# openvinotoolkit/openvino_tokenizers

Hardware: AMD Instinct MI355X
Metric: input MB/s encoded (GPT-2 BPE, 512-byte strings) (higher is better)
Workload: dtype u8/int32

## Files before the change

openvino_tokenizers_amd/csrc/api_common.hpp:

```cpp
#pragma once

#include <atomic>
#include <cstdio>
#include <cstdlib>
#include <functional>

#include <hip/hip_runtime.h>

#include <algorithm>
#include <string>

#include "encode_kernels.hpp"
#include "regex_device.hpp"
#include "runtime.hpp"
#include "tables.hpp"

struct ovtk_regex_split {
    int device = 0;
    ovtk::SplitDev dev{};
    int mode = 1;
    bool invert = false;
    int max_splits = -1;
    ovtk::RegexDev regex{};
    ovtk::DevBuf r_trans, r_ascii, r_index, r_blocks, r_ctx;
// ... 479 lines not shown
                                                                : op_ + ": output ids buffer too small (" + std::to_string(st.n_out) +
                                                                      " ids, capacity " + std::to_string(out_.data_capacity) + ")");
                if (wire_.hdr || dense_on_) return OVTK_OK;
                if (direct_out_) return OVTK_OK;
                if (int rc = copy_back(out_.begins, d_begins_, size_t(n_rows_) * 4, mem_, s_)) return rc;
                if (int rc = copy_back(out_.ends, d_ends_, size_t(n_rows_) * 4, mem_, s_)) return rc;
                if (int rc = copy_back(out_.data, d_ids_, size_t(st.n_out) * 4, mem_, s_)) return rc;
                if (mem_ == OVTK_MEM_HOST) OVTK_HIP(hipStreamSynchronize(s_));
                return OVTK_OK;
            }
            small_ = false;
            if (int rc = launch()) return rc;
        }
        return set_error(OVTK_E_HIP, "workspace sizing did not converge");
    }

private:
    int launch() {
        OVTK_HIP(hipSetDevice(device_));
        Workspace& ws = *ws_.ws;
        int e = 0;
        e = e ? e : ws.row_stage.ensure(size_t(n_rows_) * 4);
        e = e ? e : ws.row_cnt.ensure(size_t(n_rows_) * 4);
        e = e ? e : ws.row_used.ensure(size_t(n_rows_) * 4);
        e = e ? e : ws.stage.ensure(size_t(stage_cap_) * 4 + 64);
        e = e ? e : ws.deferred.ensure(size_t(shard_cap_) * kShards * sizeof(DeferredPiece));
        e = e ? e : ws.exact.ensure(size_t(exact_cap_) * sizeof(ExactPiece));
        e = e ? e : ws.scratch.ensure(size_t(scratch_cap_));
        e = e ? e : ws.wave_off.ensure(size_t(grid_ * kWavesPerBlock + 1) * sizeof(long long));
        e = e ? e : ws.tiles.ensure(size_t(n_tiles_ + 1) * sizeof(long long));
        const bool fold = fold_tail_ && n_rows_ <= kFoldTailRows;
        size_t status_bytes = sizeof(RunStatus) + (fold ? size_t(n_tiles_) * 4 + 16 : 0);
        const int sp_mode = plan_.short_path_mode;
        small_ = small_ && !(plan_.short_ok && sp_mode == 2);
        const bool span_sums = plan_.short_ok && !small_ && fold && !force_long_;
        const size_t status_stride = (status_bytes + 255) & ~size_t(255);
        e = e ? e : ws.status.ensure(2 * status_stride);
        if (fold) e = e ? e : ws.gen[4].ensure(size_t(n_rows_) * 4);
        if (self_alloc_) e = e ? e : ws.gen[5].ensure(size_t(n_rows_) * 4);
        if (e) return e;
        EncodeWork w{};
        w.n_waves = grid_ * kWavesPerBlock;
        w.fold_tail = fold;
        uint8_t* const status_base = ws.status.as<uint8_t>();
        w.tile_cnt = fold ? reinterpret_cast<int32_t*>(status_base + sizeof(RunStatus)) : nullptr;
        w.row_emit = fold ? ws.gen[4].as<int32_t>() : nullptr;
        w.pending_rows = self_alloc_ ? ws.gen[5].as<int32_t>() : nullptr;
        w.out_cap = out_.data_capacity;
        w.rows_per_ticket = plan_.rows_per_ticket;
        w.wave_off = self_alloc_ ? nullptr : ws.wave_off.as<long long>();
        w.stage_region = int32_t(stage_cap_ / kShards);
        w.row_stage = ws.row_stage.as<int32_t>();
        w.row_cnt = ws.row_cnt.as<int32_t>();
        w.row_used = ws.row_used.as<int32_t>();
        w.tile_off = ws.tiles.as<long long>();
        w.stage = ws.stage.as<int32_t>();
        w.stage_cap = int32_t(stage_cap_);
        w.stage16 = plan_.stage16 ? 1 : 0;
        w.deferred = ws.deferred.as<DeferredPiece>();
        w.shard_cap = int32_t(std::min<int64_t>(shard_cap_, INT32_MAX / kShards));
        w.exact = ws.exact.as<ExactPiece>();
        w.exact_cap = int32_t(exact_cap_);
        w.scratch = ws.scratch.as<uint8_t>();
        w.scratch_cap = uint32_t(std::min<int64_t>(scratch_cap_, 0xFFFFFFF0ll));
        w.status = ws.status.as<RunStatus>();
        phase_ = 0;

        if (small_ && fold) {
            w.small = 1;
            const int blocks = std::max(1, std::min((n_rows_ + kWavesPerBlock - 1) / kWavesPerBlock, kSmallRows / kWavesPerBlock));
            w.n_waves = blocks * kWavesPerBlock;
            w.out_ids = d_ids_;
            w.out_begins = d_begins_;
            w.out_ends = d_ends_;
            w.host_status = ws.host_status;
            w.status_words = int32_t(status_bytes / 4);
            if (ws.clean_status != w.status || ws.clean_bytes < status_bytes || ws.clean_after_lease + 1 != ws.lease_count)
                OVTK_HIP(hipMemsetAsync(w.status, 0, status_bytes, s_));
            ws.clean_status = nullptr;
            pending_clean_ = w.status;
            pending_clean_bytes_ = status_bytes;
            std::memset(ws.host_status, 0, sizeof(RunStatus));
            ws.host_status->flags = kFlagDidNotRun;
            middle_(ws, d_in_, w, blocks);
            OVTK_HIP(hipEventRecord(ws.done, s_));
            return OVTK_OK;
        }
        ws.clean_status = nullptr;
        ws.status_half ^= 1;
        uint8_t* mine = status_base + size_t(ws.status_half) * status_stride;
        uint8_t* other = status_base + size_t(ws.status_half ^ 1) * status_stride;
        w.status = reinterpret_cast<RunStatus*>(mine);
        w.tile_cnt = fold ? reinterpret_cast<int32_t*>(mine + sizeof(RunStatus)) : nullptr;
        w.next_status = reinterpret_cast<RunStatus*>(other);
        w.tile_sums = fold && (n_tiles_ <= kTileSumTiles || span_sums) ? 1 : 0;
        w.host_status = ws.host_status;
        w.status_words = int32_t(status_bytes / 4);
        if (ws.zeroed_status != mine || ws.zeroed_bytes < status_bytes || ws.zeroed_after_lease + 1 != ws.lease_count)
            OVTK_HIP(hipMemsetAsync(w.status, 0, status_bytes, s_));
        ws.zeroed_status = nullptr;
        std::memset(ws.host_status, 0, sizeof(RunStatus));
        ws.host_status->flags = kFlagDidNotRun;
        if (!self_alloc_)
            OVTK_LAUNCH(ws.marks, "prep_rows", prep_rows_kernel, std::min(grid_, kTicketBlocks), kBlockThreads, s_, d_in_, mul_, w);
        w.launch_mask = kLaunchAll;
        if (span_sums) {
            w.span_sums = 1;
            w.skip_mask = sp_mode == 2 ? (kSkipPending | kSkipMerge) : ((expect_pending_ ? 0 : kSkipPending) | (expect_merge_ ? 0 : kSkipMerge));
            w.launch_mask = kLaunchSpan | ((w.skip_mask & kSkipPending) ? 0 : kLaunchPending) | ((w.skip_mask & kSkipMerge) ? 0 : kLaunchMerge);
            w.merge_hint = int32_t(std::min<int64_t>(merge_hint_, INT32_MAX));
            w_ = w;
            phase_ = 1;
        }
        middle_(ws, d_in_, w, grid_);
        return launch_tail(ws, w, other, status_bytes);
    }

    int launch_phase2(const RunStatus& st) {
        OVTK_HIP(hipSetDevice(device_));
        Workspace& ws = *ws_.ws;
        const bool pending_now = (w_.skip_mask & kSkipPending) && st.n_pending > 0;
        if (pending_now && !(w_.skip_mask & kSkipMerge)) {
            force_long_ = true;
            return launch();
        }
        EncodeWork w = w_;
        w.merge_hint = st.n_unresolved;
        w.launch_mask = (pending_now ? kLaunchPending : 0) | ((w_.skip_mask & kSkipMerge) ? kLaunchMerge : 0);
        w.skip_mask = pending_now || !(w_.skip_mask & kSkipPending) ? 0 : kSkipPending;
        static_assert(offsetof(RunStatus, width_ticket) == offsetof(RunStatus, width) + 4, "width and width_ticket are cleared together");
        OVTK_HIP(hipMemsetAsync(&w.status->width, 0, 8, s_));
        OVTK_HIP(hipMemsetAsync(&w.status->flags, 0, 4, s_));
        OVTK_HIP(hipMemsetAsync(&w.status->n_out, 0, 4, s_));
        std::memset(ws.host_status, 0, sizeof(RunStatus));
        ws.host_status->flags = kFlagDidNotRun;
        middle_(ws, d_in_, w, grid_);
        phase_ = 2;
        return launch_tail(ws, w, zeroed_other_, zeroed_other_bytes_);
    }

    int launch_tail(Workspace& ws, EncodeWork& w, const void* other, size_t status_bytes) {
        if (!w.fold_tail)
            OVTK_LAUNCH(ws.marks, "count_scan", count_scan_kernel, std::min((n_tiles_ + 3) / 4, kTicketBlocks), kBlockThreads, s_,
                        n_rows_, w, (long long)out_.data_capacity);
        int split = 1;
        if (!dense_on_ && !wire_.hdr) {
            const long long ids_per_item = (long long)kCompactRows * (in_.strings.n_chars / std::max<long long>(1, n_rows_)) / 4;
            while (split < 16 && ids_per_item >= 2048ll * split && (long long)(n_rows_ / kCompactRows) * split * 2 <= std::max<long long>((long long)device_cu_count(device_) * 64, 1024)) split *= 2;
        }
        w.compact_split = split;
        const long long units = ((long long)n_rows_ + kCompactRows - 1) / kCompactRows * split;
        const int cgrid = int(std::max<long long>(1, std::min<long long>((units + kWavesPerBlock - 1) / kWavesPerBlock, (long long)device_cu_count(device_) * 16)));
        const RaggedSink rsink{d_ids_, d_begins_, d_ends_};
        with_bool(plan_.stage16, [&](auto s16) {
            constexpr bool S16 = decltype(s16)::value;
            if (pair_on_) {
                PairDenseSink pair = pair_;
                pair.row_cnt = w.row_cnt;
                pair.n = n_rows_ / 2;
                OVTK_LAUNCH(ws.marks, "pair_width", pair_width_kernel, std::min(64, (pair.n + kBlockThreads - 1) / kBlockThreads), kBlockThreads, s_, n_rows_, w, pair);
                OVTK_LAUNCH(ws.marks, "compact", (compact_kernel<PairDenseSink, S16>), cgrid, kBlockThreads, s_, n_rows_, w, pair);
            } else if (dense_on_) {
                OVTK_LAUNCH(ws.marks, "row_width", row_width_kernel, std::min(64, (n_rows_ + kBlockThreads - 1) / kBlockThreads), kBlockThreads, s_, n_rows_, w, dense_);
                OVTK_LAUNCH(ws.marks, "compact", (compact_kernel<DenseSink, S16>), cgrid, kBlockThreads, s_, n_rows_, w, dense_);
            } else if (wire_.hdr) OVTK_LAUNCH(ws.marks, "compact", (compact_kernel<WireSink, S16>), cgrid, kBlockThreads, s_, n_rows_, w, wire_);
            else OVTK_LAUNCH(ws.marks, "compact", (compact_kernel<RaggedSink, S16>), cgrid, kBlockThreads, s_, n_rows_, w, rsink);
        });
        pending_zeroed_ = other;
        pending_zeroed_bytes_ = status_bytes;
        zeroed_other_ = other;
        zeroed_other_bytes_ = status_bytes;
        OVTK_HIP(hipEventRecord(ws.done, s_));
        return OVTK_OK;
    }

    int device_;
    std::string op_;
    ovtk_ragged_strings in_;
    const uint8_t* skips_;
    int mul_;
    ovtk_ragged_i32_out out_;
    int mem_, in_mem_;
    bool direct_out_ = false;
    std::shared_ptr<void> keep_;
    std::vector<std::shared_ptr<WorkspaceLease>> others_;
    std::function<int()> front_check_;
    hipStream_t s_;
    Middle middle_;
    bool self_alloc_;
    EncodePlan plan_;
    WorkspaceLease ws_;
    bool fold_tail_;
    bool small_ok_ = false, small_ = false;
    bool expect_pending_ = false, expect_merge_ = true, force_long_ = false;
    int64_t merge_hint_ = -1;
    int phase_ = 0;
    EncodeWork w_{};
    const void* zeroed_other_ = nullptr;
    size_t zeroed_other_bytes_ = 0;
    const void* pending_zeroed_ = nullptr;
    size_t pending_zeroed_bytes_ = 0;
    const void* pending_clean_ = nullptr;
    size_t pending_clean_bytes_ = 0;
    WireSink wire_{};
    DenseSink dense_{};
    bool dense_on_ = false;
    PairDenseSink pair_{};
    bool pair_on_ = false;
    std::function<void(const RunStatus&)> on_status_;
    RowsIn d_in_{};
    int n_rows_ = 0, grid_ = 0, n_tiles_ = 0;
    int64_t stage_cap_ = 0, shard_cap_ = 0, exact_cap_ = 0, scratch_cap_ = 0;
    int32_t *d_begins_ = nullptr, *d_ends_ = nullptr, *d_ids_ = nullptr;
};

template <class Middle>
std::unique_ptr<RowsRun<std::decay_t<Middle>>> make_rows_run(int device, const char* op, const ovtk_ragged_strings* in,
                                                             const uint8_t* skips, int mul, const ovtk_ragged_i32_out* out, int mem,
                                                             hipStream_t s, Middle&& middle, const EncodePlan* plan = nullptr) {
    return std::make_unique<RowsRun<std::decay_t<Middle>>>(device, op, in, skips, mul, out, mem, s, std::forward<Middle>(middle), plan);
}

inline int pair_sink_from_params(const char* op, const ovtk_ragged_strings* in, int64_t n_first, const ovtk_pair_dense_params* p, int32_t* out_ids,
                                 uint8_t* out_mask, int32_t* out_type_ids, int64_t capacity, PairDenseSink& d) {
    const std::string name(op);
    if (!p || !out_ids || !in || capacity < 0) return set_error(OVTK_E_ARG, name + ": null argument");
    if (n_first < 0 || in->n_rows - n_first != n_first)
        return set_error(OVTK_E_ARG, name + ": the one call takes as many second rows as first ones (" + std::to_string(n_first) + " + " +
                                         std::to_string(in->n_rows - n_first) +
                                         "); 1 against n or an empty second input: the two-call form (the encode on all rows, then ovtk_encode_tail_run over the halves)");
    if (p->n_front < 0 || p->n_between < 0 || p->n_behind < 0 || (p->n_front && !p->front) || (p->n_between && !p->between) ||
        (p->n_behind && !p->behind) || p->max_length < 0)
        return set_error(OVTK_E_ARG, name + ": bad constant ids or max_length < 0");
    if (p->n_front > kDenseAffix || p->n_between > kDenseAffix || p->n_behind > kDenseAffix)
        return set_error(OVTK_E_UNSUPPORTED, name + ": at most 4 constant ids in front / between / behind");
    if (p->trunc_mode < 0 || p->trunc_mode > 2) return set_error(OVTK_E_ARG, name + ": Unknown truncation mode: " + std::to_string(p->trunc_mode));
    d = PairDenseSink{};
    d.ids = out_ids;
    d.mask = out_mask;
    d.types = out_type_ids;
    d.capacity = capacity;
    d.n = int32_t(n_first);
    d.max_length = p->max_length;
    d.trunc_left = p->trunc_left ? 1 : 0;
    d.mode = p->trunc_mode;
    d.pad_right = p->pad_right ? 1 : 0;
    d.pad_value = p->pad_value;
    d.type_pad = p->type_pad_value;
    d.target_dim = p->target_dim;
    d.n_front = p->n_front;
    d.n_between = p->n_between;
    d.n_behind = p->n_behind;
    for (int i = 0; i < d.n_front; ++i) d.front[i] = p->front[i];
    for (int i = 0; i < d.n_between; ++i) d.between[i] = p->between[i];
    for (int i = 0; i < d.n_behind; ++i) d.behind[i] = p->behind[i];
    for (int i = 0; i < 5; ++i) d.type_ids[i] = p->type_ids[i];
    return OVTK_OK;
}
inline int pair_rows_without_text(const PairDenseSink& d, int device, hipStream_t s, ovtk_pending& p) {
    const int32_t len = d.n_front + d.n_between + d.n_behind, T = d.target_dim >= 0 ? d.target_dim : (d.n > 0 ? len : 0);
    *p.dense_width = T;
    if (int64_t(d.n) * T > d.capacity) {
        p.late_rc = OVTK_E_CAPACITY;
        p.late_msg = "encode_pair_dense: dense outputs too small (row width " + std::to_string(T) + ")";
        return OVTK_OK;
    }
    if (T <= 0 || d.n <= 0) return OVTK_OK;
    const size_t cells = size_t(d.n) * size_t(T);
    std::vector<int32_t> ids(cells, d.pad_value), types(d.types ? cells : 0, d.type_pad);
    std::vector<uint8_t> mask(d.mask ? cells : 0, 0);
    const int col0 = d.pad_right ? 0 : std::max(0, T - len);
    for (int64_t r = 0; r < d.n; ++r)
        for (int k = 0; k < len && col0 + k < T; ++k) {
            const bool f = k < d.n_front, b = !f && k < d.n_front + d.n_between;
            const size_t at = size_t(r) * size_t(T) + size_t(col0 + k);
            ids[at] = f ? d.front[k] : (b ? d.between[k - d.n_front] : d.behind[k - d.n_front - d.n_between]);
            if (d.types) types[at] = f ? d.type_ids[0] : (b ? d.type_ids[2] : d.type_ids[4]);
            if (d.mask) mask[at] = 1;
        }
    OVTK_HIP(hipSetDevice(device));
    OVTK_HIP(hipMemcpyAsync(d.ids, ids.data(), cells * 4, hipMemcpyHostToDevice, s));
    if (d.mask) OVTK_HIP(hipMemcpyAsync(d.mask, mask.data(), cells, hipMemcpyHostToDevice, s));
    if (d.types) OVTK_HIP(hipMemcpyAsync(d.types, types.data(), cells * 4, hipMemcpyHostToDevice, s));
    OVTK_HIP(hipStreamSynchronize(s));
    return OVTK_OK;
}

template <class Middle>
int run_rows_to_ids(int device, const char* op, const ovtk_ragged_strings* in, const uint8_t* skips, int mul,
                    ovtk_ragged_i32_out* out, int mem, hipStream_t s, Middle&& middle) {
    auto run = make_rows_run(device, op, in, skips, mul, out, mem, s, std::forward<Middle>(middle));
    if (int rc = run->start()) return rc;
    return run->finish(out);
}

}
```

openvino_tokenizers_amd/csrc/encode_kernels.hpp:

```cpp
#pragma once

#include <cstddef>
#include <type_traits>

#include "bpe_device.hpp"
#include "device_common.hpp"
#include "scan_kernels.hpp"
#include "split_device.hpp"
#include "split_seq_device.hpp"

namespace ovtk {

struct RowsIn {
    const int32_t* ragged_begins;
    const int32_t* ragged_ends;
    int32_t n_rows;
    const int32_t* begins;
    const int32_t* ends;
    int32_t n_strings;
    const uint8_t* chars;
    int64_t n_chars;
    const uint8_t* skips;
};

// ... 1211 lines not shown
        }
    }
    __device__ __forceinline__ void finish(int, const RunStatus*) const {}
};
static __global__ __launch_bounds__(kBlockThreads) void row_width_kernel(int n_rows, EncodeWork w, DenseSink d) {
    int m = 0;
    if (d.target_dim < 0) {
        for (int r = int(blockIdx.x) * kBlockThreads + int(threadIdx.x); r < n_rows; r += int(gridDim.x) * kBlockThreads) {
            const int c = w.row_cnt[r];
            const int len = (c < d.max_length ? c : d.max_length) + d.n_pre + d.n_suf;
            m = len > m ? len : m;
        }
        m = wave_max(m);
        if (lane_id() == 0 && m > 0) atomicMax(&w.status->width, m);
    } else if (blockIdx.x == 0 && threadIdx.x == 0) {
        w.status->width = d.target_dim;
    }
    if (!last_block_done(&w.status->width_ticket, gridDim.x, false)) return;
    if (threadIdx.x == 0) {
        const int T = __hip_atomic_load(&w.status->width, __ATOMIC_RELAXED, __HIP_MEMORY_SCOPE_AGENT);
        if ((long long)T * n_rows > d.capacity) atomicOr(&w.status->flags, kFlagOutCapacity);
    }
}
struct PairDenseSink {
    int32_t* ids;
    uint8_t* mask;
    int32_t* types;
    int64_t capacity;
    const int32_t* row_cnt;
    int32_t n;
    int32_t max_length;
    int32_t trunc_left;
    int32_t mode;
    int32_t pad_right, pad_value, type_pad;
    int32_t target_dim;
    int32_t n_front, n_between, n_behind;
    int32_t front[kDenseAffix], between[kDenseAffix], behind[kDenseAffix];
    int32_t type_ids[5];
    int32_t T;
    __device__ __forceinline__ void start(const RunStatus* st) { T = st->width; }
    __device__ __forceinline__ int32_t front_at(int k) const { return k == 0 ? front[0] : (k == 1 ? front[1] : (k == 2 ? front[2] : front[3])); }
    __device__ __forceinline__ int32_t between_at(int k) const { return k == 0 ? between[0] : (k == 1 ? between[1] : (k == 2 ? between[2] : between[3])); }
    __device__ __forceinline__ int32_t behind_at(int k) const { return k == 0 ? behind[0] : (k == 1 ? behind[1] : (k == 2 ? behind[2] : behind[3])); }
    __device__ __forceinline__ void kept(int32_t fl, int32_t sl, int32_t& keep_f, int32_t& keep_s) const {
        const int32_t m = max_length;
        keep_f = fl;
        keep_s = sl;
        if (fl + sl > m) {
            const int32_t half = m / 2, half_up = m / 2 + m % 2;
            if (mode == 0) keep_f = fl > m ? m : fl;
            else if (mode == 1) keep_s = sl > m ? m : sl;
            else if (fl >= half_up && sl <= half) keep_f = m - sl;
            else if (fl < half_up && sl > half) keep_s = m - fl;
            else {
                keep_f = half + (m % 2) * (fl >= sl);
                keep_s = half + (m % 2) * (fl < sl);
            }
        }
    }
    __device__ __forceinline__ int col0_of(int len) const { return pad_right ? 0 : (T > len ? T - len : 0); }
    __device__ __forceinline__ void row(int, int, int) const {}
    __device__ __forceinline__ void id(int r, int cnt, int j, int, int32_t v) const {
        const bool second = r >= n;
        const int i = second ? r - n : r;
        const int32_t other = row_cnt[second ? i : r + n];
        int32_t kf, ks;
        kept(second ? other : cnt, second ? cnt : other, kf, ks);
        const int keep = second ? ks : kf, first = trunc_left ? cnt - keep : 0;
        if (j < first || j >= first + keep) return;
        const int len = n_front + kf + n_between + ks + n_behind;
        const int col = col0_of(len) + n_front + (second ? kf + n_between : 0) + (j - first);
        if (col < T) ids[(long long)i * T + col] = v;
    }
    __device__ __forceinline__ void row_done(int r, int cnt) const {
        if (r >= n) return;
        int32_t kf, ks;
        kept(cnt, row_cnt[r + n], kf, ks);
        const int a1 = n_front, a2 = a1 + kf, a3 = a2 + n_between, a4 = a3 + ks, len = a4 + n_behind;
        const int col0 = col0_of(len);
        for (int c = lane_id(); c < T; c += kWave) {
            const int k = c - col0;
            const bool inside = k >= 0 && k < len;
            const long long at = (long long)r * T + c;
            if (mask) mask[at] = inside ? uint8_t(1) : uint8_t(0);
            if (types)
                types[at] = !inside ? type_pad
                                    : (k < a1 ? type_ids[0] : (k < a2 ? type_ids[1] : (k < a3 ? type_ids[2] : (k < a4 ? type_ids[3] : type_ids[4]))));
            if (!inside) ids[at] = pad_value;
            else if (k < a1) ids[at] = front_at(k);
            else if (k >= a2 && k < a3) ids[at] = between_at(k - a2);
            else if (k >= a4) ids[at] = behind_at(k - a4);
        }
    }
    __device__ __forceinline__ void finish(int, const RunStatus*) const {}
};
static __global__ __launch_bounds__(kBlockThreads) void pair_width_kernel(int n_rows, EncodeWork w, PairDenseSink d) {
    const int n = n_rows / 2;
    int m = 0;
    if (d.target_dim < 0) {
        for (int r = int(blockIdx.x) * kBlockThreads + int(threadIdx.x); r < n; r += int(gridDim.x) * kBlockThreads) {
            int32_t kf, ks;
            d.kept(w.row_cnt[r], w.row_cnt[r + n], kf, ks);
            const int len = d.n_front + kf + d.n_between + ks + d.n_behind;
            m = len > m ? len : m;
        }
        m = wave_max(m);
        if (lane_id() == 0 && m > 0) atomicMax(&w.status->width, m);
    } else if (blockIdx.x == 0 && threadIdx.x == 0) {
        w.status->width = d.target_dim;
    }
    if (!last_block_done(&w.status->width_ticket, gridDim.x, false)) return;
    if (threadIdx.x == 0) {
        const int T = __hip_atomic_load(&w.status->width, __ATOMIC_RELAXED, __HIP_MEMORY_SCOPE_AGENT);
        if ((long long)T * n > d.capacity) atomicOr(&w.status->flags, kFlagOutCapacity);
    }
}
template <class Sink>
struct is_dense_sink { static constexpr bool value = std::is_same<Sink, DenseSink>::value || std::is_same<Sink, PairDenseSink>::value; };
struct WireSink {
    int32_t* hdr;
    int32_t* ends;
    void* ids;
    int32_t pad_ids, max_rows, id_bytes;
    __device__ __forceinline__ void start(const RunStatus*) {}
    __device__ __forceinline__ void row(int r, int, int e) const { ends[r] = e; }
    __device__ __forceinline__ void row_done(int, int) const {}
    __device__ __forceinline__ void id(int, int, int, int pos, int32_t v) const {
        if (pos >= pad_ids) return;
        if (id_bytes == 2) static_cast<uint16_t*>(ids)[pos] = uint16_t(v);
        else static_cast<int32_t*>(ids)[pos] = v;
    }
    __device__ __forceinline__ void finish(int n_rows, const RunStatus* st) const {
        if (blockIdx.x != 0) return;
        if (threadIdx.x == 0) {
            hdr[0] = st->n_out;
            hdr[1] = n_rows;
            hdr[2] = hdr[3] = 0;
        }
        for (int r = n_rows + int(threadIdx.x); r < max_rows; r += kBlockThreads) ends[r] = 0;
    }
};

template <bool S16>
__device__ __forceinline__ int32_t stage_get_t(const EncodeWork& w, int pos) {
    if (S16) {
        const uint32_t x = reinterpret_cast<const uint16_t*>(w.stage)[pos];
        return x == 0xFFFFu ? kEmptyId : int32_t(x);
    }
    return w.stage[pos];
}
constexpr int kFlatIds = kWave * 8;
struct __attribute__((packed, aligned(1))) FlatBytes16 { uint32_t d[4]; };
struct __attribute__((packed, aligned(1))) FlatBytes8 { uint32_t d[2]; };
template <bool S16>
__device__ __forceinline__ void flat_copy(const uint8_t* stage_bytes, int total_used, bool plain, int32_t* out, int32_t* buf, int part, int split) {
    constexpr int E = S16 ? 8 : 4;
    const int l = lane_id();
    auto fetch = [&](int off) -> FlatBytes16 {
        const int idx = off + l * E;
        if (idx < total_used) return *reinterpret_cast<const FlatBytes16*>(stage_bytes + idx * (S16 ? 2 : 4));
        return FlatBytes16{{0u, 0u, 0u, 0u}};
    };
    if (plain) {
        constexpr int U = 2;
        for (int off0 = part * (U * kWave * 4); off0 < total_used; off0 += split * (U * kWave * 4)) {
            uint32_t x[U][4];
#pragma unroll
            for (int u = 0; u < U; ++u) {
                const int idx = off0 + (u * kWave + l) * 4;
                x[u][0] = x[u][1] = x[u][2] = x[u][3] = 0u;
                if (idx < total_used) {
                    if (S16) {
                        const FlatBytes8 r = *reinterpret_cast<const FlatBytes8*>(stage_bytes + idx * 2);
                        x[u][0] = r.d[0] & 0xFFFFu; x[u][1] = r.d[0] >> 16; x[u][2] = r.d[1] & 0xFFFFu; x[u][3] = r.d[1] >> 16;
                    } else {
                        const FlatBytes16 r = *reinterpret_cast<const FlatBytes16*>(stage_bytes + idx * 4);
                        x[u][0] = r.d[0]; x[u][1] = r.d[1]; x[u][2] = r.d[2]; x[u][3] = r.d[3];
                    }
                }
            }
#pragma unroll
            for (int u = 0; u < U; ++u) {
                const int idx = off0 + (u * kWave + l) * 4;
                const int n_here = total_used - idx;
                if (n_here >= 4) {
                    *reinterpret_cast<FlatBytes16*>(out + idx) = FlatBytes16{{x[u][0], x[u][1], x[u][2], x[u][3]}};
                } else {
                    if (n_here > 0) out[idx] = int32_t(x[u][0]);
                    if (n_here > 1) out[idx + 1] = int32_t(x[u][1]);
                    if (n_here > 2) out[idx + 2] = int32_t(x[u][2]);
                }
            }
        }
        return;
    }
    FlatBytes16 v = fetch(0);
    for (int off = 0; off < total_used; off += kWave * E) {
        const FlatBytes16 nxt = fetch(off + kWave * E);
        const int n_here = total_used - (off + l * E);
        int32_t e[E];
        uint32_t valid = 0;
#pragma unroll
        for (int i = 0; i < E; ++i) {
            if (S16) {
                const uint32_t x = (v.d[i >> 1] >> (16 * (i & 1))) & 0xFFFFu;
                e[i] = int32_t(x);
                if (i < n_here && x != 0xFFFFu) valid |= 1u << i;
            } else {
                e[i] = int32_t(v.d[i]);
                if (i < n_here && e[i] != kEmptyId) valid |= 1u << i;
            }
        }
        const int c = __popc(valid);
        const int incl = wave_incl_sum(c);
        int at = incl - c;
#pragma unroll
        for (int i = 0; i < E; ++i)
            if ((valid >> i) & 1u) buf[at++] = e[i];
        const int total = wave_readlane(incl, kWave - 1);
        wave_sync();
        for (int t = 4 * l; t < total; t += 4 * kWave) {
            if (t + 4 <= total) {
                *reinterpret_cast<FlatBytes16*>(out + t) = *reinterpret_cast<const FlatBytes16*>(buf + t);
            } else {
                for (int i = t; i < total; ++i) out[i] = buf[i];
            }
        }
        out += total;
        v = nxt;
        wave_sync();
    }
}
template <bool S16>
__device__ __forceinline__ bool compact_flat(const EncodeWork& w, const RaggedSink& sink, int32_t* buf, const int (&cnt)[4], const int (&o)[4],
                                             const int (&base)[4], const int (&used)[4], int row0, int part, int split) {
    const int l = lane_id();
    const int total_used = used[0] + used[1] + used[2] + used[3];
    if (used[0] < 0 || used[1] < 0 || used[2] < 0 || used[3] < 0 || base[1] != base[0] + used[0] || base[2] != base[1] + used[1] ||
        base[3] != base[2] + used[2])
        return false;
    const bool plain = total_used == cnt[0] + cnt[1] + cnt[2] + cnt[3];
    if (part != 0 && !plain) return true;
    if (l < 4 && part == 0) {
        const int oo = l == 0 ? o[0] : (l == 1 ? o[1] : (l == 2 ? o[2] : o[3])), cc = l == 0 ? cnt[0] : (l == 1 ? cnt[1] : (l == 2 ? cnt[2] : cnt[3]));
        sink.row(row0 + l, oo, oo + cc);
    }
    flat_copy<S16>(reinterpret_cast<const uint8_t*>(w.stage) + (long long)base[0] * (S16 ? 2 : 4), total_used, plain, sink.ids + o[0], buf, part, split);
    return true;
}

template <class Sink, bool S16 = false>
__device__ __forceinline__ void compact_body(int n_rows, const EncodeWork& w, Sink sink, bool solo = false, int32_t* flat_buf = nullptr,
                                             uint32_t more_flags = 0u) {
    if ((w.status->flags | more_flags) & (kFatalFlags | kFlagOutCapacity | kFlagDeferOverflow | kFlagExactOverflow | kFlagScratchOverflow |
                                         kFlagTailPending))
        return;
    if ((w.skip_mask & kSkipPending) && w.status->n_pending != 0) return;
    if (w.skip_mask & kSkipMerge) {
        const int mine = lane_id() < kShards ? __hip_atomic_load(&w.status->shard_count[lane_id() * kCounterStride], __ATOMIC_RELAXED, __HIP_MEMORY_SCOPE_AGENT) : 0;
        if (__ballot(mine != 0)) return;
    }
    sink.start(w.status);
    const int l = lane_id();
    const int n_waves = (solo ? 1 : int(gridDim.x)) * kWavesPerBlock;
    constexpr int kSubs = kRowTile / kCompactRows;
    const int n_items = ((n_rows + kRowTile - 1) / kRowTile) * kSubs;
    const int split = std::is_same<Sink, RaggedSink>::value && !solo && w.compact_split > 1 ? w.compact_split : 1;
    for (int unit = (solo ? 0 : int(blockIdx.x)) * kWavesPerBlock + wave_in_block(); unit < n_items * split; unit += n_waves) {
        const int item = unit / split, part = unit % split;
        const int tile = item / kSubs, sub = item % kSubs;
        const int rj = tile * kRowTile + l;
        const bool have = rj < n_rows;
        const int c = have ? w.row_cnt[rj] : 0;
        const int sv = have ? w.row_stage[rj] : 0;
        const int uv = have ? w.row_used[rj] : 0;
        long long toff;
        if constexpr (is_dense_sink<Sink>::value) {
            toff = 0;
        } else if (w.tile_sums && !solo) {
            int acc = 0;
            const int whole = tile >> 4, rest = tile & 15;
            for (int g0 = 0; g0 < whole; g0 += kWave) {
                const int g = g0 + l;
                int4 v[4];
#pragma unroll
                for (int u = 0; u < 4; ++u) v[u] = g < whole ? *reinterpret_cast<const int4*>(w.tile_cnt + 16 * g + 4 * u) : int4{0, 0, 0, 0};
#pragma unroll
                for (int u = 0; u < 4; ++u) acc += (v[u].x + v[u].y) + (v[u].z + v[u].w);
            }
            acc += l < rest ? w.tile_cnt[16 * whole + l] : 0;
            toff = wave_sum(acc);
        } else {
            toff = w.tile_off[tile];
        }
        const int incl = wave_incl_sum(c);
        int cnt[kCompactRows], o[kCompactRows], base[kCompactRows], used[kCompactRows];
        int32_t v[kCompactRows][kCompactChunks];
#pragma unroll
        for (int q = 0; q < kCompactRows; ++q) {
            const int j = sub * kCompactRows + q;
            cnt[q] = wave_readlane(c, j);
            o[q] = int(toff + (wave_readlane(incl, j) - cnt[q]));
            base[q] = wave_readlane(sv, j);
            used[q] = wave_readlane(uv, j);
        }
        if constexpr (std::is_same<Sink, RaggedSink>::value) {
            if (w.tile_sums && !solo && (long long)o[kCompactRows - 1] + cnt[kCompactRows - 1] > w.out_cap) continue;
        }
        if constexpr (std::is_same<Sink, RaggedSink>::value && kCompactRows == 4) {
            const int row0 = tile * kRowTile + sub * kCompactRows;
            if (flat_buf && row0 + kCompactRows <= n_rows && compact_flat<S16>(w, sink, flat_buf, cnt, o, base, used, row0, part, split)) continue;
        }
        if (part != 0) continue;
#pragma unroll
        for (int q = 0; q < kCompactRows; ++q)
#pragma unroll
            for (int k = 0; k < kCompactChunks; ++k)
                v[q][k] = (k * kWave + l < used[q]) ? stage_get_t<S16>(w, base[q] + k * kWave + l) : kEmptyId;
#pragma unroll
        for (int q = 0; q < kCompactRows; ++q) {
            const int row = tile * kRowTile + sub * kCompactRows + q;
            if (row >= n_rows) break;
            if (l == 0) sink.row(row, o[q], o[q] + cnt[q]);
            int run = 0;
#pragma unroll
            for (int k = 0; k < kCompactChunks; ++k) {
                if (k * kWave < used[q]) {
                    const unsigned long long m = __ballot(v[q][k] != kEmptyId);
                    if (v[q][k] != kEmptyId) {
                        const int j = run + rank_below(m);
                        sink.id(row, cnt[q], j, o[q] + j, v[q][k]);
                    }
                    run += __popcll(m);
                }
            }
            for (int b = kCompactChunks * kWave; b < used[q]; b += kWave) {
                const int x = (b + l < used[q]) ? stage_get_t<S16>(w, base[q] + b + l) : kEmptyId;
                const unsigned long long m = __ballot(x != kEmptyId);
                if (x != kEmptyId) {
                    const int j = run + rank_below(m);
                    sink.id(row, cnt[q], j, o[q] + j, x);
                }
                run += __popcll(m);
            }
            sink.row_done(row, cnt[q]);
        }
    }
    sink.finish(n_rows, w.status);
}

template <class Sink, bool S16 = false>
static __global__ __launch_bounds__(kBlockThreads) void compact_kernel(int n_rows, EncodeWork w, Sink sink) {
    if (w.next_status && blockIdx.x == 0) {
        const uint32_t* src = reinterpret_cast<const uint32_t*>(w.status);
        uint32_t* dst = reinterpret_cast<uint32_t*>(w.host_status);
        constexpr int kHead = int(offsetof(RunStatus, shard_count) / 4);
        constexpr int kShard0 = kHead;
        for (int i = int(threadIdx.x); i < kHead + kShards; i += kBlockThreads) {
            const int at = i < kHead ? i : kShard0 + (i - kHead) * kCounterStride;
            if (w.tile_sums && (at == int(offsetof(RunStatus, n_out) / 4) || at == int(offsetof(RunStatus, flags) / 4))) continue;
            __hip_atomic_store(dst + at, __hip_atomic_load(src + at, __ATOMIC_RELAXED, __HIP_MEMORY_SCOPE_AGENT), __ATOMIC_RELAXED, __HIP_MEMORY_SCOPE_SYSTEM);
        }
        uint32_t* nxt = reinterpret_cast<uint32_t*>(w.next_status);
        for (int i = int(threadIdx.x); i < w.status_words; i += kBlockThreads) nxt[i] = 0u;
    }
    __shared__ int32_t flat_all[std::is_same<Sink, RaggedSink>::value ? kWavesPerBlock * kFlatIds : 1];
    __shared__ uint32_t over_s;
    if (threadIdx.x == 0) over_s = 0u;
    if (w.tile_sums && blockIdx.x == 0) {
        __shared__ long long total_s[kWavesPerBlock];
        const int n_tiles = (n_rows + kRowTile - 1) / kRowTile;
        long long acc = 0;
        for (int i = int(threadIdx.x); i < n_tiles; i += kBlockThreads) acc += w.tile_cnt[i];
#pragma unroll
        for (int d = kWave / 2; d > 0; d >>= 1) acc += __shfl_xor(acc, d);
        if (lane_id() == 0) total_s[wave_in_block()] = acc;
        __syncthreads();
        if (threadIdx.x == 0) {
            long long total = 0;
            for (int k = 0; k < kWavesPerBlock; ++k) total += total_s[k];
            const int32_t n_out = total > INT32_MAX ? INT32_MAX : int32_t(total);
            const uint32_t over = total > w.out_cap ? kFlagOutCapacity : 0u;
            w.status->n_out = n_out;
            if (w.next_status) {
                __hip_atomic_store(&w.host_status->n_out, n_out, __ATOMIC_RELAXED, __HIP_MEMORY_SCOPE_SYSTEM);
                __hip_atomic_store(&w.host_status->flags, __hip_atomic_load(&w.status->flags, __ATOMIC_RELAXED, __HIP_MEMORY_SCOPE_AGENT) | over,
                                   __ATOMIC_RELAXED, __HIP_MEMORY_SCOPE_SYSTEM);
            }
            if (over) atomicOr(&w.status->flags, over);
            over_s = over;
        }
    }
    __syncthreads();
    compact_body<Sink, S16>(n_rows, w, sink, false, std::is_same<Sink, RaggedSink>::value ? flat_all + wave_in_block() * kFlatIds : nullptr, over_s);
}

template <int MODE, bool NARROW>
static __global__ __launch_bounds__(kBlockThreads) void encode_small_kernel(RowsIn in, SplitDev sp, BpeDev T, EncodeWork w) {
    lookup_body<MODE, false>(in, sp, T, w);
    if (!last_block_done(&w.status->ticket[1], gridDim.x)) return;
    merge_body<NARROW>(in, T, w, in.n_rows, w.out_cap, true);
    __syncthreads();
    if (threadIdx.x == 0) publish_release();
    __syncthreads();
    publish_acquire();
    if (w.stage16) compact_body<RaggedSink, true>(in.n_rows, w, RaggedSink{w.out_ids, w.out_begins, w.out_ends}, true);
    else compact_body<RaggedSink, false>(in.n_rows, w, RaggedSink{w.out_ids, w.out_begins, w.out_ends}, true);
    __syncthreads();
    uint32_t* src = reinterpret_cast<uint32_t*>(w.status);
    uint32_t* dst = reinterpret_cast<uint32_t*>(w.host_status);
    constexpr int kHead = int(offsetof(RunStatus, shard_count) / 4);
    for (int i = int(threadIdx.x); i < w.status_words; i += kBlockThreads) {
        const uint32_t v = __hip_atomic_load(src + i, __ATOMIC_RELAXED, __HIP_MEMORY_SCOPE_AGENT);
        if (i <= kHead) __hip_atomic_store(dst + i, v, __ATOMIC_RELAXED, __HIP_MEMORY_SCOPE_SYSTEM);
        src[i] = 0;
    }
}

template <int WRITE, bool LLAMA3 = false>
static __global__ __launch_bounds__(kBlockThreads) void split_kernel(RowsIn in, SplitDev sp, int max_splits, EncodeWork w,
                                                                     int32_t* out_rb, int32_t* out_re,
                                                                     int32_t* out_begins, int32_t* out_ends,
                                                                     uint8_t* out_skips) {
    __shared__ WaveScratch ws_all[kWavesPerBlock];
    if (w.status->flags & (kFlagRange | kFlagOutCapacity)) return;
    WaveScratch& ws = ws_all[wave_in_block()];
    const int l = lane_id();
    const int n_waves = int(gridDim.x) * kWavesPerBlock;
    for (int row = int(blockIdx.x) * kWavesPerBlock + wave_in_block(); row < in.n_rows; row += n_waves) {
        int count = 0;
        int total = 0;
        const int o = WRITE == 2 ? w.row_stage[row] : (WRITE ? int(row_output_offset(w, in.n_rows, row, total)) : 0);
        if (WRITE == 1 && l == 0) {
            out_rb[row] = o;
            out_re[row] = o + total;
        }
        for (int col = in.ragged_begins[row]; col < in.ragged_ends[row]; ++col) {
            const int sb = in.begins[col], se = in.ends[col];
            if (in.skips && in.skips[col]) {
                if (WRITE && l == 0) {
                    out_begins[o + count] = sb;
                    out_ends[o + count] = se;
                    if (out_skips) out_skips[o + count] = 1;
                }
                ++count;
                continue;
            }
            int in_string = 0;
            auto emit = [&](int idx, int b, int e) {
                if (!WRITE) return;
                out_begins[o + count + idx] = sb + b;
                out_ends[o + count + idx] = (idx == max_splits) ? se : sb + e;
                if (out_skips) out_skips[o + count + idx] = 0;
            };
            scan_string<(LLAMA3 ? kScanLlama3 : kScanGeneric)>(
                ws, sp, in.chars + sb, se - sb, in.chars, in.chars + in.n_chars,
                [&](int np, int c0, int, int) {
                    for (int jb = 0; jb < np; jb += kWave) {
                        const int j = jb + l;
                        const bool keep = j < np && !(ws.pstart[j] & kPieceDropped);
                        const unsigned long long km = __ballot(keep);
                        if (keep)
                            emit(in_string + rank_below(km), c0 + int(ws.pstart[j] & kPiecePosMask),
                                 c0 + int(ws.pstart[j + 1] & kPiecePosMask));
                        in_string += __popcll(km);
                    }
                },
                [&](int b, int e, bool dropped) {
                    if (dropped) return;
                    if (l == 0) emit(in_string, b, e);
                    in_string += 1;
                });
            count += in_string;
        }
        if (WRITE != 1 && l == 0) w.row_cnt[row] = count;
    }
}

template <int WRITE>
static __global__ __launch_bounds__(kBlockThreads) void special_split_kernel(RowsIn in, SpecialDev T, EncodeWork w,
                                                                             int32_t* out_rb, int32_t* out_re,
                                                                             int32_t* out_begins, int32_t* out_ends,
                                                                             uint8_t* out_skips) {
    if (w.status->flags & (kFlagRange | kFlagOutCapacity)) return;
    const int row = int(blockIdx.x) * kBlockThreads + int(threadIdx.x);
    const bool valid = row < in.n_rows;
    int o = 0;
    if (WRITE) {
        const int cnt = valid ? w.row_cnt[row] : 0;
        const int incl = wave_incl_sum(cnt);
        o = int(w.tile_off[row / kRowTile < (in.n_rows + kRowTile - 1) / kRowTile ? row / kRowTile : 0]) + incl - cnt;
        if (valid) {
            out_rb[row] = o;
            out_re[row] = o + cnt;
        }
    }
    if (!valid) return;
    int count = 0;
    auto put = [&](int b, int e, int skip) {
        if (WRITE) {
            out_begins[o + count] = b;
            out_ends[o + count] = e;
            out_skips[o + count] = uint8_t(skip);
        }
        ++count;
    };
    for (int col = in.ragged_begins[row]; col < in.ragged_ends[row]; ++col) {
        const int sb = in.begins[col], se = in.ends[col];
        if (in.skips && in.skips[col]) {
            put(sb, se, 1);
            continue;
        }
        const uint8_t* s = in.chars + sb;
        const int slen = se - sb;
        int start = 0, mb = 0, gb = 0, ge = 0, me = 0;
        if (!string_may_hold_token(T, s, slen)) {
            if (slen > 0) put(sb, se, 0);
            continue;
        }
        while (start < slen && special_next_match(T, special_tabs(T), s, slen, start, mb, gb, ge, me)) {
            if (start < mb) put(sb + start, sb + mb, 0);
            put(sb + gb, sb + ge, 1);
            start = me;
        }
        if (start < slen) put(sb + start, sb + slen, 0);
    }
    if (!WRITE) w.row_cnt[row] = count;
}

static __global__ __launch_bounds__(kBlockThreads) void special_sparse_kernel(RowsIn in, SpecialDev T_in, RunStatus* status, long long cap,
                                                                              int32_t* out_rb, int32_t* out_re, int32_t* out_begins,
                                                                              int32_t* out_ends, uint8_t* out_skips) {
    constexpr int kLdsTokens = 64, kLdsChars = 2048, kLdsGroups = 8;
    __shared__ int32_t tb_s[kLdsTokens], te_s[kLdsTokens], gf_s[kLdsGroups + 1];
    __shared__ uint8_t gfl_s[kLdsGroups];
    __shared__ __attribute__((aligned(16))) uint8_t tc_s[kLdsChars];
    if (T_in.n_groups <= kLdsGroups && T_in.n_tokens <= kLdsTokens && T_in.n_tok_chars <= kLdsChars) {
        for (int i = int(threadIdx.x); i < T_in.n_tokens; i += kBlockThreads) {
            tb_s[i] = T_in.tok_begins[i];
            te_s[i] = T_in.tok_ends[i];
        }
        for (int i = int(threadIdx.x); i <= T_in.n_groups; i += kBlockThreads) gf_s[i] = T_in.group_first[i];
        for (int i = int(threadIdx.x); i < T_in.n_groups; i += kBlockThreads) gfl_s[i] = T_in.group_flags[i];
        for (int i = int(threadIdx.x); i < T_in.n_tok_chars; i += kBlockThreads) tc_s[i] = T_in.tok_chars[i];
        __syncthreads();
    }
    const SpecialDev& T = T_in;
// ... 155 lines not shown
```

Measured before the change: 522,400.

## Add stretched compact kernel assigning many rows per wave for span front

Adds a compact_stretch_kernel that lets each wave handle up to a full wave's worth of rows. It computes output offsets with a wave prefix sum over per-row counts plus a vectorized sum of preceding tile counts. When the rows' staged ids are contiguous, it does a single wide flat copy with a larger unroll; otherwise it falls back to per-row ballot compaction. It is selected only for the ragged span-front path with tile sums and split of 1. The aim is to cut per-row wave overhead and launch underutilization in the compact stage, at the cost of redundant tile-count summation per wave and more code paths.

```diff
diff --git a/openvino_tokenizers_amd/csrc/api_common.hpp b/openvino_tokenizers_amd/csrc/api_common.hpp
--- a/openvino_tokenizers_amd/csrc/api_common.hpp
+++ b/openvino_tokenizers_amd/csrc/api_common.hpp
@@ -655,9 +655,20 @@
         const long long units = ((long long)n_rows_ + kCompactRows - 1) / kCompactRows * split;
         const int cgrid = int(std::max<long long>(1, std::min<long long>((units + kWavesPerBlock - 1) / kWavesPerBlock, (long long)device_cu_count(device_) * 16)));
         const RaggedSink rsink{d_ids_, d_begins_, d_ends_};
+        int stretch_rows = 0;
+        if (!dense_on_ && !wire_.hdr && w.tile_sums && split == 1 && plan_.front == kFrontSpan && (w.launch_mask & kLaunchSpan)) {
+            int32_t rows = 0;
+            rows_grid(d_in_.n_rows, grid_, rows);
+            if (rows >= 1 && rows <= kWave) stretch_rows = rows;
+        }
         with_bool(plan_.stage16, [&](auto s16) {
             constexpr bool S16 = decltype(s16)::value;
-            if (pair_on_) {
+            if (stretch_rows) {
+                w.rows_per_wave = stretch_rows;
+                const long long items = ((long long)n_rows_ + stretch_rows - 1) / stretch_rows;
+                const int sgrid = int(std::max<long long>(1, std::min<long long>((items + kWavesPerBlock - 1) / kWavesPerBlock, (long long)device_cu_count(device_) * 16)));
+                OVTK_LAUNCH(ws.marks, "compact", (compact_stretch_kernel<S16>), sgrid, kBlockThreads, s_, n_rows_, w, rsink);
+            } else if (pair_on_) {
                 PairDenseSink pair = pair_;
                 pair.row_cnt = w.row_cnt;
                 pair.n = n_rows_ / 2;
diff --git a/openvino_tokenizers_amd/csrc/encode_kernels.hpp b/openvino_tokenizers_amd/csrc/encode_kernels.hpp
--- a/openvino_tokenizers_amd/csrc/encode_kernels.hpp
+++ b/openvino_tokenizers_amd/csrc/encode_kernels.hpp
@@ -1387,7 +1387,7 @@
 constexpr int kFlatIds = kWave * 8;
 struct __attribute__((packed, aligned(1))) FlatBytes16 { uint32_t d[4]; };
 struct __attribute__((packed, aligned(1))) FlatBytes8 { uint32_t d[2]; };
-template <bool S16>
+template <bool S16, int U = 2>
 __device__ __forceinline__ void flat_copy(const uint8_t* stage_bytes, int total_used, bool plain, int32_t* out, int32_t* buf, int part, int split) {
     constexpr int E = S16 ? 8 : 4;
     const int l = lane_id();
@@ -1397,7 +1397,6 @@
         return FlatBytes16{{0u, 0u, 0u, 0u}};
     };
     if (plain) {
-        constexpr int U = 2;
         for (int off0 = part * (U * kWave * 4); off0 < total_used; off0 += split * (U * kWave * 4)) {
             uint32_t x[U][4];
 #pragma unroll
@@ -1482,6 +1481,71 @@
     }
     flat_copy<S16>(reinterpret_cast<const uint8_t*>(w.stage) + (long long)base[0] * (S16 ? 2 : 4), total_used, plain, sink.ids + o[0], buf, part, split);
     return true;
+}
+
+__device__ __forceinline__ bool compact_nothing_to_write(const EncodeWork& w, uint32_t more_flags) {
+    if ((w.status->flags | more_flags) & (kFatalFlags | kFlagOutCapacity | kFlagDeferOverflow | kFlagExactOverflow | kFlagScratchOverflow |
+                                         kFlagTailPending))
+        return true;
+    if ((w.skip_mask & kSkipPending) && w.status->n_pending != 0) return true;
+    if (w.skip_mask & kSkipMerge) {
+        const int mine = lane_id() < kShards ? __hip_atomic_load(&w.status->shard_count[lane_id() * kCounterStride], __ATOMIC_RELAXED, __HIP_MEMORY_SCOPE_AGENT) : 0;
+        if (__ballot(mine != 0)) return true;
+    }
+    return false;
+}
+__device__ __forceinline__ int tiles_in_front(const EncodeWork& w, int tile, int acc = 0) {
+    const int l = lane_id();
+    const int whole = tile >> 4, rest = tile & 15;
+    for (int g0 = 0; g0 < whole; g0 += kWave) {
+        const int g = g0 + l;
+        int4 v[4];
+#pragma unroll
+        for (int u = 0; u < 4; ++u) v[u] = g < whole ? *reinterpret_cast<const int4*>(w.tile_cnt + 16 * g + 4 * u) : int4{0, 0, 0, 0};
+#pragma unroll
+        for (int u = 0; u < 4; ++u) acc += (v[u].x + v[u].y) + (v[u].z + v[u].w);
+    }
+    acc += l < rest ? w.tile_cnt[16 * whole + l] : 0;
+    return wave_sum(acc);
+}
+template <class Sink, bool S16>
+__device__ __forceinline__ void compact_rows(const EncodeWork& w, Sink sink, int row0, int row_end, const int (&cnt)[kCompactRows],
+                                             const int (&o)[kCompactRows], const int (&base)[kCompactRows], const int (&used)[kCompactRows]) {
+    const int l = lane_id();
+    int32_t v[kCompactRows][kCompactChunks];
+#pragma unroll
+    for (int q = 0; q < kCompactRows; ++q)
+#pragma unroll
+        for (int k = 0; k < kCompactChunks; ++k)
+            v[q][k] = (k * kWave + l < used[q]) ? stage_get_t<S16>(w, base[q] + k * kWave + l) : kEmptyId;
+#pragma unroll
+    for (int q = 0; q < kCompactRows; ++q) {
+        const int row = row0 + q;
+        if (row >= row_end) break;
+        if (l == 0) sink.row(row, o[q], o[q] + cnt[q]);
+        int run = 0;
+#pragma unroll
+        for (int k = 0; k < kCompactChunks; ++k) {
+            if (k * kWave < used[q]) {
+                const unsigned long long m = __ballot(v[q][k] != kEmptyId);
+                if (v[q][k] != kEmptyId) {
+                    const int j = run + rank_below(m);
+                    sink.id(row, cnt[q], j, o[q] + j, v[q][k]);
+                }
+                run += __popcll(m);
+            }
+        }
+        for (int b = kCompactChunks * kWave; b < used[q]; b += kWave) {
+            const int x = (b + l < used[q]) ? stage_get_t<S16>(w, base[q] + b + l) : kEmptyId;
+            const unsigned long long m = __ballot(x != kEmptyId);
+            if (x != kEmptyId) {
+                const int j = run + rank_below(m);
+                sink.id(row, cnt[q], j, o[q] + j, x);
+            }
+            run += __popcll(m);
+        }
+        sink.row_done(row, cnt[q]);
+    }
 }
 
 template <class Sink, bool S16 = false>
@@ -1584,8 +1648,7 @@
     sink.finish(n_rows, w.status);
 }
 
-template <class Sink, bool S16 = false>
-static __global__ __launch_bounds__(kBlockThreads) void compact_kernel(int n_rows, EncodeWork w, Sink sink) {
+__device__ __forceinline__ uint32_t compact_report(int n_rows, const EncodeWork& w) {
     if (w.next_status && blockIdx.x == 0) {
         const uint32_t* src = reinterpret_cast<const uint32_t*>(w.status);
         uint32_t* dst = reinterpret_cast<uint32_t*>(w.host_status);
@@ -1599,7 +1662,6 @@
         uint32_t* nxt = reinterpret_cast<uint32_t*>(w.next_status);
         for (int i = int(threadIdx.x); i < w.status_words; i += kBlockThreads) nxt[i] = 0u;
     }
-    __shared__ int32_t flat_all[std::is_same<Sink, RaggedSink>::value ? kWavesPerBlock * kFlatIds : 1];
     __shared__ uint32_t over_s;
     if (threadIdx.x == 0) over_s = 0u;
     if (w.tile_sums && blockIdx.x == 0) {
@@ -1627,7 +1689,62 @@
         }
     }
     __syncthreads();
-    compact_body<Sink, S16>(n_rows, w, sink, false, std::is_same<Sink, RaggedSink>::value ? flat_all + wave_in_block() * kFlatIds : nullptr, over_s);
+    return over_s;
+}
+
+template <class Sink, bool S16 = false>
+static __global__ __launch_bounds__(kBlockThreads) void compact_kernel(int n_rows, EncodeWork w, Sink sink) {
+    __shared__ int32_t flat_all[std::is_same<Sink, RaggedSink>::value ? kWavesPerBlock * kFlatIds : 1];
+    const uint32_t over = compact_report(n_rows, w);
+    compact_body<Sink, S16>(n_rows, w, sink, false, std::is_same<Sink, RaggedSink>::value ? flat_all + wave_in_block() * kFlatIds : nullptr, over);
+}
+
+constexpr int kStretchGroups = 4;
+template <bool S16>
+static __global__ __launch_bounds__(kBlockThreads) void compact_stretch_kernel(int n_rows, EncodeWork w, RaggedSink sink) {
+    __shared__ int32_t flat_all[kWavesPerBlock * kFlatIds];
+    const uint32_t over = compact_report(n_rows, w);
+    if (compact_nothing_to_write(w, over)) return;
+    const int l = lane_id();
+    const int R = w.rows_per_wave;
+    const int n_items = (n_rows + R - 1) / R;
+    const int n_waves = int(gridDim.x) * kWavesPerBlock;
+    int32_t* const buf = flat_all + wave_in_block() * kFlatIds;
+    for (int item = int(blockIdx.x) * kWavesPerBlock + wave_in_block(); item < n_items; item += n_waves) {
+        const int row0 = item * R;
+        const int nr = n_rows - row0 < R ? n_rows - row0 : R;
+        const int tile = row0 / kRowTile, in_front = row0 % kRowTile;
+        const bool mine = l < nr;
+        const int c = mine ? w.row_cnt[row0 + l] : 0;
+        const int sv = mine ? w.row_stage[row0 + l] : 0;
+        const int uv = mine ? w.row_used[row0 + l] : 0;
+        const int toff = tiles_in_front(w, tile, l < in_front ? w.row_cnt[tile * kRowTile + l] : 0);
+        const int incl = wave_incl_sum(c);
+        const int total_cnt = wave_readlane(incl, kWave - 1);
+        if ((long long)toff + total_cnt > w.out_cap) continue;
+        const int o = toff + (incl - c);
+        const int next_sv = int(lane_next(uint32_t(sv)));
+        const bool flat = __ballot(mine && (uv < 0 || (l + 1 < nr && next_sv != sv + uv))) == 0ull;
+        if (flat) {
+            if (mine) sink.row(row0 + l, o, o + c);
+            const int total_used = wave_sum(uv);
+            flat_copy<S16, kStretchGroups>(reinterpret_cast<const uint8_t*>(w.stage) + (long long)wave_readlane(sv, 0) * (S16 ? 2 : 4), total_used,
+                                           total_used == total_cnt, sink.ids + toff, buf, 0, 1);
+            continue;
+        }
+        for (int q0 = 0; q0 < nr; q0 += kCompactRows) {
+            int cnt[kCompactRows], oo[kCompactRows], base[kCompactRows], used[kCompactRows];
+#pragma unroll
+            for (int q = 0; q < kCompactRows; ++q) {
+                const int j = q0 + q;
+                cnt[q] = wave_readlane(c, j);
+                oo[q] = wave_readlane(o, j);
+                base[q] = wave_readlane(sv, j);
+                used[q] = wave_readlane(uv, j);
+            }
+            compact_rows<RaggedSink, S16>(w, sink, row0 + q0, row0 + nr, cnt, oo, base, used);
+        }
+    }
 }
 
 template <int MODE, bool NARROW>
```

New measurement: 563,500 (median of 6 runs). +7.9%, better.
